# vitoplantamura/OnnxStream

Measured on AMD Instinct MI355X. Metric: sd15_unet_step_latency_ms+images_per_sec_512x512_20step, higher is better.
Workload: dtype f16

## Files before the change

onnxstream_amd/csrc/osg_tchain.hip:

```cpp
#include "osg_common.h"

#include <cstdlib>
#include <type_traits>

namespace osg_tb {

struct TailParams {
    const f16 *a1, *x0;
    const f16 *wo1, *bo1;
    const f16 *g2, *be2;
    float eps2;
    const f16 *wq2, *bq2;
    const f16 *kp, *vtp;
    float sc_log2e;
    int Tk;
    const f16 *wo2, *bo2;
    const f16 *g3, *be3;
    float eps3;
    const f16 *w1, *b1, *w2, *b2;
    const f16 *wpo, *bpo, *xin;
    f16 *out, *out2;
    long ldo, ldo2;
    int M, rows_per_img, heads;
    int pf_sleep0, pf_sleep;
    f16* dbg[8];
};

typedef __attribute__((address_space(3))) void* lds_ptr;

__device__ __forceinline__ void lds_barrier() {
    asm volatile("s_waitcnt lgkmcnt(0)" ::: "memory");
    __builtin_amdgcn_s_barrier();
}


template <int I, int N, typename Fn>
__device__ __forceinline__ void static_for_impl(Fn&& f) {
    if constexpr (I < N) {
        f(std::integral_constant<int, I>{});
        static_for_impl<I + 1, N>(f);
    }
}
template <int N, typename Fn>
__device__ __forceinline__ void static_for(Fn&& f) { static_for_impl<0, N>(f); }

template <int RT>
constexpr int kTileBytes = RT * 2048;

template <int RT>
__device__ __forceinline__ int img_off(int m, int n) { return (n >> 6) * kTileBytes<RT> + m * 128 + ((((n & 63) >> 3) ^ (m & 7)) << 4) + (n & 7) * 2; }

typedef unsigned u32x4 __attribute__((ext_vector_type(4)));
__device__ __forceinline__ f16x8 ldb(__amdgpu_buffer_rsrc_t rs, unsigned lo, int so) {
    return __builtin_bit_cast(f16x8, __builtin_amdgcn_raw_buffer_load_b128(rs, lo, so, 0));
}
template <int NT>
__device__ __forceinline__ void load_b(f16x8 (&b)[10], __amdgpu_buffer_rsrc_t rs, unsigned lo, int so, int kstep) {
#pragma unroll
    for (int ks = 0; ks < 2; ks++)
#pragma unroll
        for (int j = 0; j < NT; j++) b[ks * 5 + j] = ldb(rs, lo, so + j * 256 + ks * kstep);
}
__device__ __forceinline__ void load_b_geglu(f16x8 (&b)[10], __amdgpu_buffer_rsrc_t rs, unsigned lo, int so, int kstep, int gate_off) {
#pragma unroll
    for (int ks = 0; ks < 2; ks++) {
#pragma unroll
        for (int j = 0; j < 4; j++) b[ks * 5 + j] = ldb(rs, lo, so + (j & 1) * 256 + (j >> 1) * gate_off + ks * kstep);
        b[ks * 5 + 4] = b[ks * 5 + 3];
    }
}

template <int RT, int NT>
__device__ __forceinline__ void mma_ktile(const char* At, int a_rd, const f16x8 (&b)[10], f32x4 (&acc)[RT][NT]) {
#pragma unroll
    for (int ks = 0; ks < 2; ks++) {
        f16x8 a[RT];
#pragma unroll
        for (int i = 0; i < RT; i++) a[i] = *reinterpret_cast<const f16x8*>(At + ((a_rd + i * 2048) ^ (ks << 6)));
#pragma unroll
        for (int j = 0; j < NT; j++)
#pragma unroll
            for (int i = 0; i < RT; i++) acc[i][j] = __builtin_amdgcn_mfma_f32_16x16x32_f16(b[ks * 5 + j], a[i], acc[i][j], 0, 0, 0);
    }
}

template <int RT, int KT, int NT, int SS, int NS, typename Load, typename Next, typename Mark>
__device__ __forceinline__ void gemm_stage(const char* A, int a_rd, f16x8 (&bq)[NS][10], f32x4 (&acc)[RT][NT], Load&& load, Next&& next, Mark&& mark) {
    static_for<KT>([&](auto tc) __attribute__((always_inline)) {
        constexpr int t = decltype(tc)::value;
        mark(t);
        if constexpr (t + NS - 1 < KT) load(bq[(SS + t + NS - 1) % NS], t + NS - 1);
        else next(bq[(SS + t + NS - 1) % NS], t + NS - 1 - KT);
        __builtin_amdgcn_sched_barrier(0);
        mma_ktile<RT, NT>(A + t * kTileBytes<RT>, a_rd, bq[(SS + t) % NS], acc);
        __builtin_amdgcn_sched_barrier(0);
    });
}

template <int RT, int KT, int NT, int SS, int NS, typename Load, typename Next>
__device__ __forceinline__ void gemm_stage(const char* A, int a_rd, f16x8 (&bq)[NS][10], f32x4 (&acc)[RT][NT], Load&& load, Next&& next) {
    gemm_stage<RT, KT, NT, SS, NS>(A, a_rd, bq, acc, load, next, [](int) __attribute__((always_inline)) {});
}

template <int RT, int KT, int NT, typename After, typename Mark>
__device__ __forceinline__ void square_stage(const char* A, int a_rd, f16x8 (&bs)[KT][10], f32x4 (&acc)[RT][NT], After&& after, Mark&& mark) {
    static_for<KT>([&](auto tc) __attribute__((always_inline)) {
        constexpr int t = decltype(tc)::value;
        mark(t);
        __builtin_amdgcn_sched_barrier(0);
        mma_ktile<RT, NT>(A + t * kTileBytes<RT>, a_rd, bs[t], acc);
        __builtin_amdgcn_sched_barrier(0);
        after(bs[t], t);
    });
}

template <int RT, int NT>
__device__ __forceinline__ void zero_acc(f32x4 (&acc)[RT][NT]) {
#pragma unroll
    for (int i = 0; i < RT; i++)
#pragma unroll
        for (int j = 0; j < NT; j++) acc[i][j] = f32x4{0.f, 0.f, 0.f, 0.f};
}

template <int RT, int NT, bool RES>
__device__ __forceinline__ void epi_to_lds(const f32x4 (&acc)[RT][NT], const char* bias, int nb, const char* res, char* dst, int lane) {
    const int l16 = lane & 15, g4 = (lane >> 4) * 4;
#pragma unroll
    for (int j = 0; j < NT; j++) {
        const int n = nb + j * 16 + g4;
        const f16x4 bv = *reinterpret_cast<const f16x4*>(bias + n * 2);
#pragma unroll
        for (int i = 0; i < RT; i++) {
            const int off = img_off<RT>(i * 16 + l16, n);
            f16x4 rv = f16x4{0, 0, 0, 0};
            if constexpr (RES) rv = *reinterpret_cast<const f16x4*>(res + off);
            f16x4 o;
#pragma unroll
            for (int r = 0; r < 4; r++) o[r] = (f16)((acc[i][j][r] + (float)bv[r]) + (float)rv[r]);
            *reinterpret_cast<f16x4*>(dst + off) = o;
        }
    }
}

template <int RT, int NT, bool RES_LDS, bool OUT2>
__device__ __forceinline__ void epi_to_global(const f32x4 (&acc)[RT][NT], const char* bias, int nb, const char* res_lds, const f16x4 (&rg)[RT][NT],
                                              f16* __restrict__ out, long ldo, f16* __restrict__ out2, long ldo2, long row0, int lane) {
    const int l16 = lane & 15, g4 = (lane >> 4) * 4;
#pragma unroll
    for (int j = 0; j < NT; j++) {
        const int n = nb + j * 16 + g4;
        const f16x4 bv = *reinterpret_cast<const f16x4*>(bias + n * 2);
#pragma unroll
        for (int i = 0; i < RT; i++) {
            const int m = i * 16 + l16;
            f16x4 rv = rg[i][j];
            if constexpr (RES_LDS) rv = *reinterpret_cast<const f16x4*>(res_lds + img_off<RT>(m, n));
            f16x4 o;
#pragma unroll
            for (int r = 0; r < 4; r++) o[r] = (f16)((acc[i][j][r] + (float)bv[r]) + (float)rv[r]);
            *reinterpret_cast<f16x4*>(out + (row0 + m) * ldo + n) = o;
            if constexpr (OUT2) *reinterpret_cast<f16x4*>(out2 + (row0 + m) * ldo2 + n) = o;
        }
    }
}

template <int RT, int C>
__device__ __forceinline__ void ln_rows(const char* X, char* P, const char* gamma, const char* beta, float eps, int tid) {
    constexpr int NCH = C / 8, LPR = 16 / RT, PER = NCH / LPR;
    static_assert(NCH % LPR == 0 && (LPR == 4 || LPR == 8), "row chunks split over the lanes of a row");
    const int row = tid / LPR, part = tid % LPR;
    float v[PER][8];
    float s = 0.f;
#pragma unroll
    for (int i = 0; i < PER; i++) {
        const int c = part + LPR * i;
        const f16x8 t = *reinterpret_cast<const f16x8*>(X + (c >> 3) * kTileBytes<RT> + row * 128 + (((c & 7) ^ (row & 7)) << 4));
#pragma unroll
        for (int e = 0; e < 8; e++) { v[i][e] = (float)t[e]; s += v[i][e]; }
    }
    s += __shfl_xor(s, 1, 64);
    s += __shfl_xor(s, 2, 64);
    if constexpr (LPR == 8) s += __shfl_xor(s, 4, 64);
    const float mean = s / (float)C;
    float q = 0.f;
#pragma unroll
    for (int i = 0; i < PER; i++)
#pragma unroll
        for (int e = 0; e < 8; e++) { const float d = v[i][e] - mean; q += d * d; }
    q += __shfl_xor(q, 1, 64);
    q += __shfl_xor(q, 2, 64);
    if constexpr (LPR == 8) q += __shfl_xor(q, 4, 64);
    const float rstd = 1.0f / sqrtf(q / (float)C + eps);
#pragma unroll
    for (int i = 0; i < PER; i++) {
        const int c = part + LPR * i;
        const f16x8 gm = *reinterpret_cast<const f16x8*>(gamma + c * 16);
        const f16x8 bt = *reinterpret_cast<const f16x8*>(beta + c * 16);
        f16x8 o;
#pragma unroll
        for (int e = 0; e < 8; e++) o[e] = (f16)((v[i][e] - mean) * rstd * (float)gm[e] + (float)bt[e]);
        *reinterpret_cast<f16x8*>(P + (c >> 3) * kTileBytes<RT> + row * 128 + (((c & 7) ^ (row & 7)) << 4)) = o;
    }
}

template <int RT, int C>
__device__ __forceinline__ void dump_img(const char* img, f16* __restrict__ dst, long row0, int tid) {
    if (!dst) return;
    constexpr int NCH = C / 8;
    for (int idx = tid; idx < 16 * RT * NCH; idx += 256) {
        const int row = idx / NCH, c = idx - row * NCH;
        *reinterpret_cast<f16x8*>(dst + (row0 + row) * C + c * 8) =
            *reinterpret_cast<const f16x8*>(img + (c >> 3) * kTileBytes<RT> + row * 128 + (((c & 7) ^ (row & 7)) << 4));
    }
}

template <int RT, int D, int TKT>
__device__ __forceinline__ void cross_attention(const char* Qi, char* Oi, const f16* __restrict__ kp, const f16* __restrict__ vtp, int head0, int nheads, float c, int Tk, int lane) {
    constexpr int DS = (D + 15) / 16, DP = DS * 16, TKP = TKT * 16;
    const int l16 = lane & 15, g = lane >> 4;
    for (int hh = 0; hh < nheads; hh++) {
        const int h = head0 + hh;
        const f16* kh = kp + (long)h * TKP * DP;
        const f16* vh = vtp + (long)h * DP * TKP;
        f16x4 kf[TKT][DS], vf[DS][TKT];
#pragma unroll
        for (int tt = 0; tt < TKT; tt++)
#pragma unroll
            for (int ds = 0; ds < DS; ds++) kf[tt][ds] = *reinterpret_cast<const f16x4*>(kh + (tt * 16 + l16) * DP + ds * 16 + g * 4);
#pragma unroll
        for (int dt = 0; dt < DS; dt++)
#pragma unroll
            for (int tt = 0; tt < TKT; tt++) vf[dt][tt] = *reinterpret_cast<const f16x4*>(vh + (dt * 16 + l16) * TKP + tt * 16 + g * 4);
#pragma unroll 1
        for (int mi = 0; mi < RT; mi++) {
            const int m = mi * 16 + l16;
            f16x4 qf[DS];
#pragma unroll
            for (int ds = 0; ds < DS; ds++) {
                const int dd = ds * 16 + g * 4;
                const bool ok = dd < D;
                const f16x4 t = *reinterpret_cast<const f16x4*>(Qi + img_off<RT>(m, h * D + (ok ? dd : 0)));
                qf[ds] = ok ? t : f16x4{0, 0, 0, 0};
            }
            f32x4 s[TKT];
#pragma unroll
            for (int tt = 0; tt < TKT; tt++) {
                s[tt] = f32x4{0.f, 0.f, 0.f, 0.f};
#pragma unroll
                for (int ds = 0; ds < DS; ds++) s[tt] = __builtin_amdgcn_mfma_f32_16x16x16f16(kf[tt][ds], qf[ds], s[tt], 0, 0, 0);
            }
            float mx = -INFINITY;
#pragma unroll
            for (int tt = 0; tt < TKT; tt++)
#pragma unroll
                for (int r = 0; r < 4; r++) {
                    const float v = (tt * 16 + g * 4 + r) < Tk ? s[tt][r] * c : -INFINITY;
                    s[tt][r] = v;
                    mx = fmaxf(mx, v);
                }
            mx = fmaxf(mx, __shfl_xor(mx, 16, 64));
            mx = fmaxf(mx, __shfl_xor(mx, 32, 64));
            float sum = 0.f;
            f16x4 pf[TKT];
#pragma unroll
            for (int tt = 0; tt < TKT; tt++)
#pragma unroll
                for (int r = 0; r < 4; r++) {
                    const float e = __builtin_amdgcn_exp2f(s[tt][r] - mx);
                    sum += e;
                    pf[tt][r] = (f16)e;
                }
            sum += __shfl_xor(sum, 16, 64);
            sum += __shfl_xor(sum, 32, 64);
            const float inv = 1.0f / sum;
#pragma unroll
            for (int dt = 0; dt < DS; dt++) {
                f32x4 o = f32x4{0.f, 0.f, 0.f, 0.f};
#pragma unroll
                for (int tt = 0; tt < TKT; tt++) o = __builtin_amdgcn_mfma_f32_16x16x16f16(vf[dt][tt], pf[tt], o, 0, 0, 0);
                const int dd = dt * 16 + g * 4;
                if (dd < D) {
                    f16x4 ov;
#pragma unroll
                    for (int r = 0; r < 4; r++) ov[r] = (f16)(o[r] * inv);
                    *reinterpret_cast<f16x4*>(Oi + img_off<RT>(m, h * D + dd)) = ov;
                }
            }
        }
    }
}

__device__ __forceinline__ void touch_lines(const void* base, int rows, int row_bytes, long pitch, int tid, char* lds_dummy) {
    const int lpr = (row_bytes + 127) >> 7, n = rows * lpr;
    __amdgpu_buffer_rsrc_t rs = __builtin_amdgcn_make_buffer_rsrc((void*)base, 0, (int)((rows - 1) * pitch + row_bytes), 0x00020000);
    for (int i = tid; i < n; i += 256) {
        const int r = i / lpr, l = i - r * lpr;
        __builtin_amdgcn_raw_ptr_buffer_load_lds(rs, (lds_ptr)lds_dummy, 4, (unsigned)(r * pitch + l * 128), 0, 0, 0);
    }
}

template <int RT, int C, int D, int TKT, int NS>
__global__ __launch_bounds__(256, RT == 2 && NS == 2 ? 2 : 1) void tblock_tail_kernel(const void* a1, const void* x0, const void* wo1, const void* bo1, const void* g2, const void* be2, int M, int rows_per_img, TailParams pk) {
    TailParams p = pk;
    p.a1 = (const f16*)a1; p.x0 = (const f16*)x0; p.wo1 = (const f16*)wo1; p.bo1 = (const f16*)bo1; p.g2 = (const f16*)g2; p.be2 = (const f16*)be2; p.M = M; p.rows_per_img = rows_per_img;
    constexpr int RB = 16 * RT;
    constexpr int TB = kTileBytes<RT>;
    constexpr int KT = C / 64;
    constexpr int NTW = C / 64;
    constexpr int F = 4 * C;
    constexpr int HC = 128, NCHUNK = F / HC;
    constexpr int G2T = HC / 64;
    constexpr int PER = KT + G2T;
    constexpr int IMG = KT * TB;
    constexpr int AH = NS - 1;
    static_assert(C % 64 == 0 && NTW <= 5 && 2 * G2T * TB <= IMG && (RT == 2 || RT == 4) && (NS == 2 || NS == 3) && PER % NS == 1 && AH <= G2T && AH <= KT, "shape");
    constexpr int KS_C = 4 * C * 16, KT_C = 8 * C * 16, KS_1 = 4 * 2 * F * 16, KT_1 = 8 * 2 * F * 16;
    constexpr int GATE = F * 16;
    constexpr int CH1 = HC * 16;
    constexpr int CH2 = (HC / 8) * C * 16;
    const int tid = threadIdx.x;
    const int nblk = p.M / RB;

    if ((int)blockIdx.x >= nblk) {
        extern __shared__ __attribute__((aligned(16))) char lds_pf[];
        char* dummy = lds_pf + __builtin_amdgcn_readfirstlane(tid >> 6) * 256;
        auto nap = [&](int n) __attribute__((always_inline)) { for (; n > 0; n -= 127) __builtin_amdgcn_s_sleep(127); };
        touch_lines(p.wq2, 1, C * C * 2, 0, tid, dummy);
        {
            constexpr int DP = (D + 15) / 16 * 16;
            const int imgs = p.M / p.rows_per_img, bytes = imgs * p.heads * TKT * 16 * DP * 2;
            touch_lines(p.kp, 1, bytes, 0, tid, dummy);
            touch_lines(p.vtp, 1, bytes, 0, tid, dummy);
        }
        touch_lines(p.wo2, 1, C * C * 2, 0, tid, dummy);
        nap(p.pf_sleep0);
        for (int c = 0; c < NCHUNK; c++) {
            touch_lines((const char*)p.w1 + c * CH1, C / 8, HC * 16, 2 * F * 16, tid, dummy);
            touch_lines((const char*)p.w1 + GATE + c * CH1, C / 8, HC * 16, 2 * F * 16, tid, dummy);
            touch_lines((const char*)p.w2 + c * CH2, 1, CH2, 0, tid, dummy);
            if (c == NCHUNK / 2 && p.wpo) touch_lines(p.wpo, 1, C * C * 2, 0, tid, dummy);
            nap(p.pf_sleep);
        }
        return;
    }

    extern __shared__ __attribute__((aligned(16))) char lds[];
    char* const X = lds;
    char* const P = lds + IMG;
    char* const R = lds + 2 * IMG;
    char* const VEC = lds + 3 * IMG;
    enum { V_BO1, V_G2, V_BE2, V_BQ2, V_BO2, V_G3, V_BE3, V_B2, V_BPO, V_B1 };
    auto vec = [&](int k) __attribute__((always_inline)) { return VEC + k * (C * 2); };
    {
        const f16* src[10] = {p.bo1, p.g2, p.be2, p.bq2, p.bo2, p.g3, p.be3, p.b2, p.bpo, p.b1};
#pragma unroll
        for (int k = 0; k < 10; k++) {
            const int n16 = (k == V_B1 ? 2 * F : C) / 8;
            for (int i = tid; i < n16; i += 256) {
                f16x8 v = f16x8{0, 0, 0, 0, 0, 0, 0, 0};
                if (src[k]) v = *reinterpret_cast<const f16x8*>(src[k] + i * 8);
                *reinterpret_cast<f16x8*>(vec(k) + i * 16) = v;
            }
        }
    }
    const int lane = tid & 63;
    const int wave = __builtin_amdgcn_readfirstlane(tid >> 6);
    const int l16 = lane & 15, g = lane >> 4;
    const long row0 = (long)blockIdx.x * RB;
    const int img = (int)(row0 / p.rows_per_img);
    const int a_rd = l16 * 128 + ((g ^ (l16 & 7)) << 4);
    const int nb = wave * (C / 4);
    long long* const stamps = reinterpret_cast<long long*>(p.dbg[7]);
    auto stamp = [&](int k) __attribute__((always_inline)) { if (stamps && tid == 0) stamps[(long)blockIdx.x * 32 + k] = wall_clock64(); };
    stamp(0);

    f16x8 bq[NS][10];
    f16x8 bs[KT][10];
    const unsigned lo_c = (unsigned)((g * C + nb + l16) * 16);
    const unsigned lo_1 = (unsigned)((g * 2 * F + wave * 32 + l16) * 16);
    const __amdgpu_buffer_rsrc_t u_o1 = __builtin_amdgcn_make_buffer_rsrc((void*)p.wo1, 0, C * C * 2, 0x00020000);
    const __amdgpu_buffer_rsrc_t u_q2 = __builtin_amdgcn_make_buffer_rsrc((void*)p.wq2, 0, C * C * 2, 0x00020000);
    const __amdgpu_buffer_rsrc_t u_o2 = __builtin_amdgcn_make_buffer_rsrc((void*)p.wo2, 0, C * C * 2, 0x00020000);
    const __amdgpu_buffer_rsrc_t u_1 = __builtin_amdgcn_make_buffer_rsrc((void*)p.w1, 0, 2 * F * C * 2, 0x00020000);
    const __amdgpu_buffer_rsrc_t u_2 = __builtin_amdgcn_make_buffer_rsrc((void*)p.w2, 0, C * F * 2, 0x00020000);
    const __amdgpu_buffer_rsrc_t u_po = __builtin_amdgcn_make_buffer_rsrc((void*)p.wpo, 0, p.wpo ? C * C * 2 : 0, 0x00020000);
    const bool has_po = p.wpo != nullptr;
    auto ld_cc = [&](f16x8 (&b)[10], __amdgpu_buffer_rsrc_t rs, int t) __attribute__((always_inline)) { load_b<NTW>(b, rs, lo_c, t * KT_C, KS_C); };
    auto ld_ff = [&](f16x8 (&b)[10], int cc, int pos) __attribute__((always_inline)) {
        if (pos < KT) load_b_geglu(b, u_1, lo_1, cc * CH1 + pos * KT_1, KS_1, GATE);
        else load_b<NTW>(b, u_2, lo_c, (cc - 1) * CH2 + (pos - KT) * KT_C, KS_C);
    };

    static_for<KT>([&](auto tc) __attribute__((always_inline)) { ld_cc(bs[decltype(tc)::value], u_o1, decltype(tc)::value); });

    {
        __amdgpu_buffer_rsrc_t rsA = __builtin_amdgcn_make_buffer_rsrc((void*)(p.a1 + row0 * C), 0, RB * C * 2, 0x00020000);
        __amdgpu_buffer_rsrc_t rsX = __builtin_amdgcn_make_buffer_rsrc((void*)(p.x0 + row0 * C), 0, RB * C * 2, 0x00020000);
        const int rsub = lane >> 3, gch = (lane & 7) ^ rsub;
#pragma unroll
        for (int kt = 0; kt < KT; kt++)
#pragma unroll
            for (int qq = 0; qq < RT / 2; qq++) {
                const int q8 = qq * 4 + wave;
                const unsigned off = (unsigned)(((q8 * 8 + rsub) * C + kt * 64 + gch * 8) * 2);
                __builtin_amdgcn_raw_ptr_buffer_load_lds(rsA, (lds_ptr)(P + kt * TB + q8 * 1024), 16, off, 0, 0, 0);
                __builtin_amdgcn_raw_ptr_buffer_load_lds(rsX, (lds_ptr)(X + kt * TB + q8 * 1024), 16, off, 0, 0, 0);
            }
    }
    asm volatile("s_waitcnt vmcnt(0)" ::: "memory");
    lds_barrier();
    stamp(1);

    {
        f32x4 acc[RT][NTW];
        zero_acc(acc);
        square_stage<RT, KT, NTW>(P, a_rd, bs, acc, [&](f16x8 (&)[10], int t) __attribute__((always_inline)) { if (t < AH) ld_cc(bq[t % NS], u_q2, t); },
                              [&](int t) __attribute__((always_inline)) { stamp(16 + t); });
        stamp(21);
        epi_to_lds<RT, NTW, true>(acc, vec(V_BO1), nb, X, X, lane);
        stamp(22);
    }
    lds_barrier();
    stamp(2);
    dump_img<RT, C>(X, p.dbg[0], row0, tid);
    ln_rows<RT, C>(X, P, vec(V_G2), vec(V_BE2), p.eps2, tid);
    lds_barrier();
    stamp(3);
    dump_img<RT, C>(P, p.dbg[1], row0, tid);

    {
        f32x4 acc[RT][NTW];
        zero_acc(acc);
        gemm_stage<RT, KT, NTW, 0, NS>(P, a_rd, bq, acc, [&](f16x8 (&b)[10], int t) __attribute__((always_inline)) { ld_cc(b, u_q2, t); },
                                   [&](f16x8 (&b)[10], int j) __attribute__((always_inline)) { ld_cc(b, u_o2, j); });
        epi_to_lds<RT, NTW, false>(acc, vec(V_BQ2), nb, nullptr, R, lane);
    }
    lds_barrier();
    stamp(4);
    dump_img<RT, C>(R, p.dbg[2], row0, tid);

    {
        constexpr int DS = (D + 15) / 16, DP = DS * 16, TKP = TKT * 16;
        const int hpw = p.heads >> 2;
        const long per_img = (long)p.heads * TKP * DP;
        cross_attention<RT, D, TKT>(R, P, p.kp + img * per_img, p.vtp + img * per_img, wave * hpw, hpw, p.sc_log2e, p.Tk, lane);
    }
    lds_barrier();
    stamp(5);
    dump_img<RT, C>(P, p.dbg[3], row0, tid);

    {
        f32x4 acc[RT][NTW];
        zero_acc(acc);
        gemm_stage<RT, KT, NTW, KT, NS>(P, a_rd, bq, acc, [&](f16x8 (&b)[10], int t) __attribute__((always_inline)) { ld_cc(b, u_o2, t); },
                                    [&](f16x8 (&b)[10], int j) __attribute__((always_inline)) { ld_ff(b, 0, j); });
        epi_to_lds<RT, NTW, true>(acc, vec(V_BO2), nb, X, X, lane);
    }
    lds_barrier();
    stamp(6);
    dump_img<RT, C>(X, p.dbg[4], row0, tid);
    ln_rows<RT, C>(X, P, vec(V_G3), vec(V_BE3), p.eps3, tid);
    lds_barrier();
    stamp(7);
    dump_img<RT, C>(P, p.dbg[5], row0, tid);

    f32x4 accY[RT][NTW];
    zero_acc(accY);
    {
        constexpr int S0 = 2 * KT;
        f32x4 accG[RT][4];
        auto geglu_store = [&](int c) __attribute__((always_inline)) {
            char* H = R + (c & 1) * (G2T * TB);
#pragma unroll
            for (int jt = 0; jt < 2; jt++) {
                const int hc = wave * 32 + jt * 16 + g * 4;
                const f16x4 bv = *reinterpret_cast<const f16x4*>(vec(V_B1) + (c * HC + hc) * 2);
                const f16x4 bg = *reinterpret_cast<const f16x4*>(vec(V_B1) + (F + c * HC + hc) * 2);
#pragma unroll
                for (int i = 0; i < RT; i++) {
                    f16x4 o;
#pragma unroll
                    for (int r = 0; r < 4; r++) o[r] = (f16)((accG[i][jt][r] + (float)bv[r]) * osg_gelu_erf(accG[i][2 + jt][r] + (float)bg[r]));
                    *reinterpret_cast<f16x4*>(H + img_off<RT>(i * 16 + l16, hc)) = o;
                }
            }
        };
        zero_acc(accG);
        gemm_stage<RT, KT, 4, S0, NS>(P, a_rd, bq, accG, [&](f16x8 (&b)[10], int t) __attribute__((always_inline)) { ld_ff(b, 0, t); },
                                  [&](f16x8 (&b)[10], int j) __attribute__((always_inline)) { ld_ff(b, 1, j); });
        geglu_store(0);
        lds_barrier();
        stamp(8);
        auto ff_iter = [&](auto st, int c) __attribute__((always_inline)) {
            constexpr int ST = decltype(st)::value;
            const bool last = c == NCHUNK - 1;
            auto request = [&](f16x8 (&b)[10], int pos) __attribute__((always_inline)) {
                if (pos < PER) ld_ff(b, c, pos);
                else if (!last) ld_ff(b, c + 1, pos - PER);
                else ld_ff(b, NCHUNK, KT + pos - PER);
            };
            zero_acc(accG);
            static_for<KT>([&](auto tc) __attribute__((always_inline)) {
                constexpr int t = decltype(tc)::value;
                request(bq[(ST + t + AH) % NS], t + AH);
                __builtin_amdgcn_sched_barrier(0);
                mma_ktile<RT, 4>(P + t * TB, a_rd, bq[(ST + t) % NS], accG);
                __builtin_amdgcn_sched_barrier(0);
            });
            if (c == 3) stamp(24); else if (c == 4) stamp(28);
            const char* Hp = R + ((c - 1) & 1) * (G2T * TB);
            static_for<G2T>([&](auto uc) __attribute__((always_inline)) {
                constexpr int u = decltype(uc)::value;
                request(bq[(ST + KT + u + AH) % NS], KT + u + AH);
                __builtin_amdgcn_sched_barrier(0);
                mma_ktile<RT, NTW>(Hp + u * TB, a_rd, bq[(ST + KT + u) % NS], accY);
            });
            if (c == 3) stamp(25); else if (c == 4) stamp(29);
            geglu_store(c);
            if (c == 3) stamp(26); else if (c == 4) stamp(30);
            lds_barrier();
            if (c == 2) stamp(23); else if (c == 3) stamp(27); else if (c == 4) stamp(31);
        };
        constexpr int B0 = (S0 + KT) % NS;
        int c = 1;
        for (; c + NS <= NCHUNK; c += NS) {
            ff_iter(std::integral_constant<int, B0 % NS>{}, c);
            ff_iter(std::integral_constant<int, (B0 + 1) % NS>{}, c + 1);
            if constexpr (NS == 3) ff_iter(std::integral_constant<int, (B0 + 2) % NS>{}, c + 2);
        }
        constexpr int REM = (NCHUNK - 1) % NS;
        if constexpr (REM >= 1) ff_iter(std::integral_constant<int, B0 % NS>{}, c);
        if constexpr (REM >= 2) ff_iter(std::integral_constant<int, (B0 + 1) % NS>{}, c + 1);
        stamp(9);
        {
            constexpr int ST = (S0 + KT + (NCHUNK - 1) * PER) % NS;
            const char* Hp = R + ((NCHUNK - 1) & 1) * (G2T * TB);
            static_for<G2T>([&](auto uc) __attribute__((always_inline)) {
                constexpr int u = decltype(uc)::value;
                if constexpr (u + AH < G2T) ld_ff(bq[(ST + u + AH) % NS], NCHUNK, KT + u + AH);
                else if (has_po) ld_cc(bq[(ST + u + AH) % NS], u_po, u + AH - G2T);
                __builtin_amdgcn_sched_barrier(0);
                mma_ktile<RT, NTW>(Hp + u * TB, a_rd, bq[(ST + u) % NS], accY);
                __builtin_amdgcn_sched_barrier(0);
            });
        }
    }
    stamp(10);
    f16x4 rg[RT][NTW];
#pragma unroll
    for (int i = 0; i < RT; i++)
#pragma unroll
        for (int j = 0; j < NTW; j++) rg[i][j] = f16x4{0, 0, 0, 0};
    if (!has_po) {
        if (p.out2) epi_to_global<RT, NTW, true, true>(accY, vec(V_B2), nb, X, rg, p.out, p.ldo, p.out2, p.ldo2, row0, lane);
        else epi_to_global<RT, NTW, true, false>(accY, vec(V_B2), nb, X, rg, p.out, p.ldo, nullptr, 0, row0, lane);
        if (stamps) { asm volatile("s_waitcnt vmcnt(0)" ::: "memory"); stamp(13); }
        return;
    }
#pragma unroll
    for (int i = 0; i < RT; i++)
#pragma unroll
        for (int j = 0; j < NTW; j++) rg[i][j] = *reinterpret_cast<const f16x4*>(p.xin + (row0 + i * 16 + l16) * C + nb + j * 16 + g * 4);
    epi_to_lds<RT, NTW, true>(accY, vec(V_B2), nb, X, P, lane);
    lds_barrier();
    stamp(11);
    dump_img<RT, C>(P, p.dbg[6], row0, tid);
    {
        f32x4 acc[RT][NTW];
        zero_acc(acc);
        constexpr int SS = 2 * KT + KT + (NCHUNK - 1) * PER + G2T;
        gemm_stage<RT, KT, NTW, SS, NS>(P, a_rd, bq, acc, [&](f16x8 (&b)[10], int t) __attribute__((always_inline)) { ld_cc(b, u_po, t); },
                                    [&](f16x8 (&)[10], int) __attribute__((always_inline)) {});
        stamp(12);
        if (p.out2) epi_to_global<RT, NTW, false, true>(acc, vec(V_BPO), nb, nullptr, rg, p.out, p.ldo, p.out2, p.ldo2, row0, lane);
        else epi_to_global<RT, NTW, false, false>(acc, vec(V_BPO), nb, nullptr, rg, p.out, p.ldo, nullptr, 0, row0, lane);
        if (stamps) { asm volatile("s_waitcnt vmcnt(0)" ::: "memory"); stamp(13); }
    }
}

struct PackJob { int k_col, v_col, D, dst; };
__global__ __launch_bounds__(256) void kv_pack_kernel(const f16* __restrict__ base, long ld, int Tk, int heads, int imgs, const PackJob* __restrict__ jobs, f16* __restrict__ dst) {
    const int per_job = imgs * heads;
    const int j = blockIdx.x / per_job, ih = blockIdx.x - j * per_job, img = ih / heads, h = ih - img * heads;
    const PackJob job = jobs[j];
    const int D = job.D, DP = (D + 15) / 16 * 16, TKP = 80, NC = DP / 8;
    f16* kp = dst + job.dst + (long)ih * TKP * DP;
    f16* vtp = dst + job.dst + (long)per_job * TKP * DP + (long)ih * TKP * DP;
    const f16* k = base + job.k_col + h * D + (long)img * Tk * ld;
    const f16* v = base + job.v_col + h * D + (long)img * Tk * ld;
    for (int idx = threadIdx.x; idx < TKP * NC; idx += 256) {
        const int t = idx / NC, d0 = (idx - t * NC) * 8;
        const bool in = t < Tk && d0 < D;
        f16x8 kv = f16x8{0, 0, 0, 0, 0, 0, 0, 0}, vv = kv;
        if (in) {
            kv = *reinterpret_cast<const f16x8*>(k + (long)t * ld + d0);
            vv = *reinterpret_cast<const f16x8*>(v + (long)t * ld + d0);
        }
        *reinterpret_cast<f16x8*>(kp + t * DP + d0) = kv;
#pragma unroll
        for (int e = 0; e < 8; e++) vtp[(d0 + e) * TKP + t] = vv[e];
    }
}

__global__ __launch_bounds__(256) void kn8_pack_kernel(const f16x8* __restrict__ src, f16x8* __restrict__ dst, int N, int K8) {
    const long idx = (long)blockIdx.x * 256 + threadIdx.x;
    if (idx >= (long)N * K8) return;
    const int kc = (int)(idx / N), n = (int)(idx - (long)kc * N);
    dst[idx] = src[(long)n * K8 + kc];
}


}

extern "C" {

int osg_tblock_tail_supported(int M, int rows_per_img, int C, int heads, int Tk) {
    return C == 320 && heads == 8 && M > 0 && M % 32 == 0 && rows_per_img % 32 == 0 && Tk >= 1 && Tk <= 80;
}

size_t osg_tblock_kv_pack_elems(int imgs, int heads, int D) { return (size_t)imgs * heads * 80 * (size_t)((D + 15) / 16 * 16); }

int osg_tblock_pack_weight(osg_ctx* ctx, const void* w_nk, int N, int K, void* w_kn8) {
    if (N < 1 || K < 8 || K % 8) OSG_FAIL(ctx, "osg_tblock_pack_weight: K must be a multiple of 8");
    const long n = (long)N * (K / 8);
    hipLaunchKernelGGL(osg_tb::kn8_pack_kernel, dim3((unsigned)((n + 255) / 256)), dim3(256), 0, ctx->compute, (const f16x8*)w_nk, (f16x8*)w_kn8, N, K / 8);
    OSG_LAUNCH_CHECK(ctx);
    return 0;
}

int osg_tblock_kv_pack_jobs(osg_ctx* ctx, const void* base, long ld, int imgs, int Tk, int heads, int njobs, const int* jobs_dev, void* dst) {
    if (Tk < 1 || Tk > 80 || njobs < 1 || imgs < 1 || heads < 1 || ld % 8) OSG_FAIL(ctx, "osg_tblock_kv_pack_jobs: unsupported shape (1 <= Tk <= 80, row pitch a multiple of 8 elements; columns and head dims multiples of 8)");
    hipLaunchKernelGGL(osg_tb::kv_pack_kernel, dim3((unsigned)(njobs * imgs * heads)), dim3(256), 0, ctx->compute, (const f16*)base, ld, Tk, heads, imgs,
                       (const osg_tb::PackJob*)jobs_dev, (f16*)dst);
    OSG_LAUNCH_CHECK(ctx);
    return 0;
}

int osg_tblock_tail(osg_ctx* ctx, const osg_tblock_tail_args* a) {
    if (!osg_tblock_tail_supported(a->M, a->rows_per_img, a->C, a->heads, a->Tk)) OSG_FAIL(ctx, "osg_tblock_tail: unsupported shape (see osg_tblock_tail_supported)");
    if (!(a->scale > 0.f)) OSG_FAIL(ctx, "osg_tblock_tail: scale must be > 0");
    if (!a->a1 || !a->x0 || !a->wo1 || !a->g2 || !a->be2 || !a->wq2 || !a->kp || !a->vtp || !a->wo2 || !a->g3 || !a->be3 || !a->w1 || !a->w2 || !a->out)
        OSG_FAIL(ctx, "osg_tblock_tail: missing operand");
    if (a->wpo && !a->xin) OSG_FAIL(ctx, "osg_tblock_tail: proj_out needs its residual");
    osg_tb::TailParams p;
    p.a1 = (const f16*)a->a1; p.x0 = (const f16*)a->x0;
    p.wo1 = (const f16*)a->wo1; p.bo1 = (const f16*)a->bo1;
    p.g2 = (const f16*)a->g2; p.be2 = (const f16*)a->be2; p.eps2 = a->eps2;
    p.wq2 = (const f16*)a->wq2; p.bq2 = (const f16*)a->bq2;
    p.kp = (const f16*)a->kp; p.vtp = (const f16*)a->vtp;
    p.sc_log2e = a->scale * 1.4426950408889634f;
    p.Tk = a->Tk;
    p.wo2 = (const f16*)a->wo2; p.bo2 = (const f16*)a->bo2;
    p.g3 = (const f16*)a->g3; p.be3 = (const f16*)a->be3; p.eps3 = a->eps3;
    p.w1 = (const f16*)a->w1; p.b1 = (const f16*)a->b1; p.w2 = (const f16*)a->w2; p.b2 = (const f16*)a->b2;
    p.wpo = (const f16*)a->wpo; p.bpo = (const f16*)a->bpo; p.xin = (const f16*)a->xin;
    p.out = (f16*)a->out; p.out2 = (f16*)a->out2;
    p.ldo = a->ldo ? a->ldo : a->C; p.ldo2 = a->ldo2;
    p.M = a->M; p.rows_per_img = a->rows_per_img; p.heads = a->heads;
    for (int i = 0; i < 8; i++) p.dbg[i] = (f16*)a->dbg[i];
    static const int pfw = getenv("OSG_TBLOCK_PREFETCH") ? atoi(getenv("OSG_TBLOCK_PREFETCH")) : 8;
    static const int pfs0 = getenv("OSG_TBLOCK_PF_SLEEP0") ? atoi(getenv("OSG_TBLOCK_PF_SLEEP0")) : 100;
    static const int pfs = getenv("OSG_TBLOCK_PF_SLEEP") ? atoi(getenv("OSG_TBLOCK_PF_SLEEP")) : 60;
    p.pf_sleep0 = pfs0; p.pf_sleep = pfs;
    static const int rows_env = getenv("OSG_TBLOCK_ROWS") ? atoi(getenv("OSG_TBLOCK_ROWS")) : 0;
    int rows = a->rows_per_block == 32 || a->rows_per_block == 64 ? a->rows_per_block : rows_env == 32 || rows_env == 64 ? rows_env : (a->M / 64 < 2 * ctx->num_cu ? 32 : 64);
    if (a->rows_per_block != 0 && a->rows_per_block != 32 && a->rows_per_block != 64) OSG_FAIL(ctx, "osg_tblock_tail: rows_per_block must be 0, 32 or 64");
    if (a->M % 64 || a->rows_per_img % 64) {
        if (a->rows_per_block == 64) OSG_FAIL(ctx, "osg_tblock_tail: 64-row blocks need M and rows_per_img to be multiples of 64");
        rows = 32;
    }
    const int nblk = a->M / rows;
    const int npf = nblk >= 64 && nblk + pfw <= ctx->num_cu ? pfw : 0;
    auto launch = [&](auto kern, int smem, unsigned long long& attr_mask) -> int {
        if (osg_first_on_device(attr_mask)) {
            OSG_HIP(ctx, hipFuncSetAttribute((const void*)kern, hipFuncAttributeMaxDynamicSharedMemorySize, smem));
        }
        hipLaunchKernelGGL(kern, dim3((unsigned)(nblk + npf)), dim3(256), smem, ctx->compute, (const void*)p.a1, (const void*)p.x0, (const void*)p.wo1, (const void*)p.bo1, (const void*)p.g2, (const void*)p.be2, p.M, p.rows_per_img, p);
        return 0;
    };
    constexpr int vec_bytes = (9 * 320 + 8 * 320) * 2;
    static unsigned long long attr64 = 0, attr32 = 0, attr32n3 = 0;
    static const bool ns3 = getenv("OSG_TBLOCK_NS") && atoi(getenv("OSG_TBLOCK_NS")) == 3;
    int rc;
    if (rows == 64) rc = launch(osg_tb::tblock_tail_kernel<4, 320, 40, 5, 2>, 3 * 5 * osg_tb::kTileBytes<4> + vec_bytes, attr64);
    else if (ns3) rc = launch(osg_tb::tblock_tail_kernel<2, 320, 40, 5, 3>, 3 * 5 * osg_tb::kTileBytes<2> + vec_bytes, attr32n3);
    else rc = launch(osg_tb::tblock_tail_kernel<2, 320, 40, 5, 2>, 3 * 5 * osg_tb::kTileBytes<2> + vec_bytes, attr32);
    if (rc) return rc;
    OSG_LAUNCH_CHECK(ctx);
    osg_set_kernel(ctx, 4, rows, rows == 32 && ns3 ? 3 : 2, nblk, npf, a->wpo ? 1 : 0, a->out2 ? 1 : 0);
    return 0;
}

}
```

Baseline: 10.34.

## Split FFN chunks across two wave groups in 32-row transformer tail kernel

Adds an NG=2 variant of the fused transformer-block tail kernel with 512 threads, used by default for 32-row blocks. The second group of four waves takes odd GEGLU/FFN chunks and half the cross-attention heads, and its FFN partial accumulators are reduced through LDS into group 0. The aim is more waves per block to hide weight-streaming latency in the FFN. In exchange, the non-FFN GEMMs leave group 1 idle, there are extra barriers and a reduction step, and per-block register/LDS demand rises, which may lower occupancy.

```diff
diff --git a/onnxstream_amd/csrc/osg_tchain.hip b/onnxstream_amd/csrc/osg_tchain.hip
--- a/onnxstream_amd/csrc/osg_tchain.hip
+++ b/onnxstream_amd/csrc/osg_tchain.hip
@@ -203,11 +203,11 @@
     }
 }
 
-template <int RT, int C>
+template <int RT, int C, int NTH>
 __device__ __forceinline__ void dump_img(const char* img, f16* __restrict__ dst, long row0, int tid) {
     if (!dst) return;
     constexpr int NCH = C / 8;
-    for (int idx = tid; idx < 16 * RT * NCH; idx += 256) {
+    for (int idx = tid; idx < 16 * RT * NCH; idx += NTH) {
         const int row = idx / NCH, c = idx - row * NCH;
         *reinterpret_cast<f16x8*>(dst + (row0 + row) * C + c * 8) =
             *reinterpret_cast<const f16x8*>(img + (c >> 3) * kTileBytes<RT> + row * 128 + (((c & 7) ^ (row & 7)) << 4));
@@ -290,17 +290,18 @@
     }
 }
 
+template <int NTH>
 __device__ __forceinline__ void touch_lines(const void* base, int rows, int row_bytes, long pitch, int tid, char* lds_dummy) {
     const int lpr = (row_bytes + 127) >> 7, n = rows * lpr;
     __amdgpu_buffer_rsrc_t rs = __builtin_amdgcn_make_buffer_rsrc((void*)base, 0, (int)((rows - 1) * pitch + row_bytes), 0x00020000);
-    for (int i = tid; i < n; i += 256) {
+    for (int i = tid; i < n; i += NTH) {
         const int r = i / lpr, l = i - r * lpr;
         __builtin_amdgcn_raw_ptr_buffer_load_lds(rs, (lds_ptr)lds_dummy, 4, (unsigned)(r * pitch + l * 128), 0, 0, 0);
     }
 }
 
-template <int RT, int C, int D, int TKT, int NS>
-__global__ __launch_bounds__(256, RT == 2 && NS == 2 ? 2 : 1) void tblock_tail_kernel(const void* a1, const void* x0, const void* wo1, const void* bo1, const void* g2, const void* be2, int M, int rows_per_img, TailParams pk) {
+template <int RT, int C, int D, int TKT, int NS, int NG = 1>
+__global__ __launch_bounds__(256 * NG, RT == 2 && NS == 2 ? 2 : 1) void tblock_tail_kernel(const void* a1, const void* x0, const void* wo1, const void* bo1, const void* g2, const void* be2, int M, int rows_per_img, TailParams pk) {
     TailParams p = pk;
     p.a1 = (const f16*)a1; p.x0 = (const f16*)x0; p.wo1 = (const f16*)wo1; p.bo1 = (const f16*)bo1; p.g2 = (const f16*)g2; p.be2 = (const f16*)be2; p.M = M; p.rows_per_img = rows_per_img;
     constexpr int RB = 16 * RT;
@@ -313,7 +314,13 @@
     constexpr int PER = KT + G2T;
     constexpr int IMG = KT * TB;
     constexpr int AH = NS - 1;
+    constexpr int NTH = 256 * NG;
+    constexpr int CS = NG;
+    constexpr int NITER = NCHUNK / CS;
+    constexpr int SUMB = RT * NTW * 256 * 16;
+    constexpr int RSZ = NG == 2 ? SUMB : IMG;
     static_assert(C % 64 == 0 && NTW <= 5 && 2 * G2T * TB <= IMG && (RT == 2 || RT == 4) && (NS == 2 || NS == 3) && PER % NS == 1 && AH <= G2T && AH <= KT, "shape");
+    static_assert((NG == 1 || NG == 2) && NCHUNK % CS == 0 && RSZ >= IMG && RSZ >= NG * 2 * G2T * TB && (NG == 1 || RT == 2), "wave groups");
     constexpr int KS_C = 4 * C * 16, KT_C = 8 * C * 16, KS_1 = 4 * 2 * F * 16, KT_1 = 8 * 2 * F * 16;
     constexpr int GATE = F * 16;
     constexpr int CH1 = HC * 16;
@@ -325,20 +332,20 @@
         extern __shared__ __attribute__((aligned(16))) char lds_pf[];
         char* dummy = lds_pf + __builtin_amdgcn_readfirstlane(tid >> 6) * 256;
         auto nap = [&](int n) __attribute__((always_inline)) { for (; n > 0; n -= 127) __builtin_amdgcn_s_sleep(127); };
-        touch_lines(p.wq2, 1, C * C * 2, 0, tid, dummy);
+        touch_lines<NTH>(p.wq2, 1, C * C * 2, 0, tid, dummy);
         {
             constexpr int DP = (D + 15) / 16 * 16;
             const int imgs = p.M / p.rows_per_img, bytes = imgs * p.heads * TKT * 16 * DP * 2;
-            touch_lines(p.kp, 1, bytes, 0, tid, dummy);
-            touch_lines(p.vtp, 1, bytes, 0, tid, dummy);
-        }
-        touch_lines(p.wo2, 1, C * C * 2, 0, tid, dummy);
+            touch_lines<NTH>(p.kp, 1, bytes, 0, tid, dummy);
+            touch_lines<NTH>(p.vtp, 1, bytes, 0, tid, dummy);
+        }
+        touch_lines<NTH>(p.wo2, 1, C * C * 2, 0, tid, dummy);
         nap(p.pf_sleep0);
         for (int c = 0; c < NCHUNK; c++) {
-            touch_lines((const char*)p.w1 + c * CH1, C / 8, HC * 16, 2 * F * 16, tid, dummy);
-            touch_lines((const char*)p.w1 + GATE + c * CH1, C / 8, HC * 16, 2 * F * 16, tid, dummy);
-            touch_lines((const char*)p.w2 + c * CH2, 1, CH2, 0, tid, dummy);
-            if (c == NCHUNK / 2 && p.wpo) touch_lines(p.wpo, 1, C * C * 2, 0, tid, dummy);
+            touch_lines<NTH>((const char*)p.w1 + c * CH1, C / 8, HC * 16, 2 * F * 16, tid, dummy);
+            touch_lines<NTH>((const char*)p.w1 + GATE + c * CH1, C / 8, HC * 16, 2 * F * 16, tid, dummy);
+            touch_lines<NTH>((const char*)p.w2 + c * CH2, 1, CH2, 0, tid, dummy);
+            if (c == NCHUNK / 2 && p.wpo) touch_lines<NTH>(p.wpo, 1, C * C * 2, 0, tid, dummy);
             nap(p.pf_sleep);
         }
         return;
@@ -348,7 +355,7 @@
     char* const X = lds;
     char* const P = lds + IMG;
     char* const R = lds + 2 * IMG;
-    char* const VEC = lds + 3 * IMG;
+    char* const VEC = lds + 2 * IMG + RSZ;
     enum { V_BO1, V_G2, V_BE2, V_BQ2, V_BO2, V_G3, V_BE3, V_B2, V_BPO, V_B1 };
     auto vec = [&](int k) __attribute__((always_inline)) { return VEC + k * (C * 2); };
     {
@@ -356,7 +363,7 @@
 #pragma unroll
         for (int k = 0; k < 10; k++) {
             const int n16 = (k == V_B1 ? 2 * F : C) / 8;
-            for (int i = tid; i < n16; i += 256) {
+            for (int i = tid; i < n16; i += NTH) {
                 f16x8 v = f16x8{0, 0, 0, 0, 0, 0, 0, 0};
                 if (src[k]) v = *reinterpret_cast<const f16x8*>(src[k] + i * 8);
                 *reinterpret_cast<f16x8*>(vec(k) + i * 16) = v;
@@ -365,11 +372,14 @@
     }
     const int lane = tid & 63;
     const int wave = __builtin_amdgcn_readfirstlane(tid >> 6);
+    const int grp = NG == 2 ? wave >> 2 : 0;
+    const int w4 = NG == 2 ? wave & 3 : wave;
+    const bool g0 = grp == 0;
     const int l16 = lane & 15, g = lane >> 4;
     const long row0 = (long)blockIdx.x * RB;
     const int img = (int)(row0 / p.rows_per_img);
     const int a_rd = l16 * 128 + ((g ^ (l16 & 7)) << 4);
-    const int nb = wave * (C / 4);
+    const int nb = w4 * (C / 4);
     long long* const stamps = reinterpret_cast<long long*>(p.dbg[7]);
     auto stamp = [&](int k) __attribute__((always_inline)) { if (stamps && tid == 0) stamps[(long)blockIdx.x * 32 + k] = wall_clock64(); };
     stamp(0);
@@ -377,7 +387,7 @@
     f16x8 bq[NS][10];
     f16x8 bs[KT][10];
     const unsigned lo_c = (unsigned)((g * C + nb + l16) * 16);
-    const unsigned lo_1 = (unsigned)((g * 2 * F + wave * 32 + l16) * 16);
+    const unsigned lo_1 = (unsigned)((g * 2 * F + w4 * 32 + l16) * 16);
     const __amdgpu_buffer_rsrc_t u_o1 = __builtin_amdgcn_make_buffer_rsrc((void*)p.wo1, 0, C * C * 2, 0x00020000);
     const __amdgpu_buffer_rsrc_t u_q2 = __builtin_amdgcn_make_buffer_rsrc((void*)p.wq2, 0, C * C * 2, 0x00020000);
     const __amdgpu_buffer_rsrc_t u_o2 = __builtin_amdgcn_make_buffer_rsrc((void*)p.wo2, 0, C * C * 2, 0x00020000);
@@ -388,10 +398,10 @@
     auto ld_cc = [&](f16x8 (&b)[10], __amdgpu_buffer_rsrc_t rs, int t) __attribute__((always_inline)) { load_b<NTW>(b, rs, lo_c, t * KT_C, KS_C); };
     auto ld_ff = [&](f16x8 (&b)[10], int cc, int pos) __attribute__((always_inline)) {
         if (pos < KT) load_b_geglu(b, u_1, lo_1, cc * CH1 + pos * KT_1, KS_1, GATE);
-        else load_b<NTW>(b, u_2, lo_c, (cc - 1) * CH2 + (pos - KT) * KT_C, KS_C);
+        else load_b<NTW>(b, u_2, lo_c, (cc - CS) * CH2 + (pos - KT) * KT_C, KS_C);
     };
 
-    static_for<KT>([&](auto tc) __attribute__((always_inline)) { ld_cc(bs[decltype(tc)::value], u_o1, decltype(tc)::value); });
+    if (g0) static_for<KT>([&](auto tc) __attribute__((always_inline)) { ld_cc(bs[decltype(tc)::value], u_o1, decltype(tc)::value); });
 
     {
         __amdgpu_buffer_rsrc_t rsA = __builtin_amdgcn_make_buffer_rsrc((void*)(p.a1 + row0 * C), 0, RB * C * 2, 0x00020000);
@@ -401,20 +411,23 @@
         for (int kt = 0; kt < KT; kt++)
 #pragma unroll
             for (int qq = 0; qq < RT / 2; qq++) {
-                const int q8 = qq * 4 + wave;
+                const int q8 = qq * 4 + w4;
                 const unsigned off = (unsigned)(((q8 * 8 + rsub) * C + kt * 64 + gch * 8) * 2);
-                __builtin_amdgcn_raw_ptr_buffer_load_lds(rsA, (lds_ptr)(P + kt * TB + q8 * 1024), 16, off, 0, 0, 0);
-                __builtin_amdgcn_raw_ptr_buffer_load_lds(rsX, (lds_ptr)(X + kt * TB + q8 * 1024), 16, off, 0, 0, 0);
+                if (NG == 1 || g0) __builtin_amdgcn_raw_ptr_buffer_load_lds(rsA, (lds_ptr)(P + kt * TB + q8 * 1024), 16, off, 0, 0, 0);
+                if (NG == 1 || !g0) __builtin_amdgcn_raw_ptr_buffer_load_lds(rsX, (lds_ptr)(X + kt * TB + q8 * 1024), 16, off, 0, 0, 0);
             }
     }
     asm volatile("s_waitcnt vmcnt(0)" ::: "memory");
     lds_barrier();
     stamp(1);
 
-    {
+    if (g0) {
         f32x4 acc[RT][NTW];
         zero_acc(acc);
-        square_stage<RT, KT, NTW>(P, a_rd, bs, acc, [&](f16x8 (&)[10], int t) __attribute__((always_inline)) { if (t < AH) ld_cc(bq[t % NS], u_q2, t); },
+        square_stage<RT, KT, NTW>(P, a_rd, bs, acc, [&](f16x8 (&)[10], int t) __attribute__((always_inline)) {
+                                  constexpr int DL = NG == 2 ? 1 : 0;
+                                  if (t >= DL && t - DL < AH) ld_cc(bq[(t - DL) % NS], u_q2, t - DL);
+                              },
                               [&](int t) __attribute__((always_inline)) { stamp(16 + t); });
         stamp(21);
         epi_to_lds<RT, NTW, true>(acc, vec(V_BO1), nb, X, X, lane);
@@ -422,13 +435,13 @@
     }
     lds_barrier();
     stamp(2);
-    dump_img<RT, C>(X, p.dbg[0], row0, tid);
-    ln_rows<RT, C>(X, P, vec(V_G2), vec(V_BE2), p.eps2, tid);
+    dump_img<RT, C, NTH>(X, p.dbg[0], row0, tid);
+    if (g0) ln_rows<RT, C>(X, P, vec(V_G2), vec(V_BE2), p.eps2, tid);
     lds_barrier();
     stamp(3);
-    dump_img<RT, C>(P, p.dbg[1], row0, tid);
-
-    {
+    dump_img<RT, C, NTH>(P, p.dbg[1], row0, tid);
+
+    if (g0) {
         f32x4 acc[RT][NTW];
         zero_acc(acc);
         gemm_stage<RT, KT, NTW, 0, NS>(P, a_rd, bq, acc, [&](f16x8 (&b)[10], int t) __attribute__((always_inline)) { ld_cc(b, u_q2, t); },
@@ -437,43 +450,46 @@
     }
     lds_barrier();
     stamp(4);
-    dump_img<RT, C>(R, p.dbg[2], row0, tid);
+    dump_img<RT, C, NTH>(R, p.dbg[2], row0, tid);
 
     {
         constexpr int DS = (D + 15) / 16, DP = DS * 16, TKP = TKT * 16;
-        const int hpw = p.heads >> 2;
+        const int hpw = p.heads >> (NG == 2 ? 3 : 2);
         const long per_img = (long)p.heads * TKP * DP;
         cross_attention<RT, D, TKT>(R, P, p.kp + img * per_img, p.vtp + img * per_img, wave * hpw, hpw, p.sc_log2e, p.Tk, lane);
     }
     lds_barrier();
     stamp(5);
-    dump_img<RT, C>(P, p.dbg[3], row0, tid);
-
-    {
+    dump_img<RT, C, NTH>(P, p.dbg[3], row0, tid);
+
+    if (g0) {
         f32x4 acc[RT][NTW];
         zero_acc(acc);
         gemm_stage<RT, KT, NTW, KT, NS>(P, a_rd, bq, acc, [&](f16x8 (&b)[10], int t) __attribute__((always_inline)) { ld_cc(b, u_o2, t); },
                                     [&](f16x8 (&b)[10], int j) __attribute__((always_inline)) { ld_ff(b, 0, j); });
         epi_to_lds<RT, NTW, true>(acc, vec(V_BO2), nb, X, X, lane);
+    } else {
+        static_for<AH>([&](auto jc) __attribute__((always_inline)) { ld_ff(bq[(2 * KT + decltype(jc)::value) % NS], grp, decltype(jc)::value); });
     }
     lds_barrier();
     stamp(6);
-    dump_img<RT, C>(X, p.dbg[4], row0, tid);
-    ln_rows<RT, C>(X, P, vec(V_G3), vec(V_BE3), p.eps3, tid);
+    dump_img<RT, C, NTH>(X, p.dbg[4], row0, tid);
+    if (g0) ln_rows<RT, C>(X, P, vec(V_G3), vec(V_BE3), p.eps3, tid);
     lds_barrier();
     stamp(7);
-    dump_img<RT, C>(P, p.dbg[5], row0, tid);
+    dump_img<RT, C, NTH>(P, p.dbg[5], row0, tid);
 
     f32x4 accY[RT][NTW];
     zero_acc(accY);
     {
         constexpr int S0 = 2 * KT;
         f32x4 accG[RT][4];
+        auto hbuf = [&](int c) __attribute__((always_inline)) { return R + (NG == 2 ? grp * 2 + ((c >> 1) & 1) : c & 1) * (G2T * TB); };
         auto geglu_store = [&](int c) __attribute__((always_inline)) {
-            char* H = R + (c & 1) * (G2T * TB);
+            char* H = hbuf(c);
 #pragma unroll
             for (int jt = 0; jt < 2; jt++) {
-                const int hc = wave * 32 + jt * 16 + g * 4;
+                const int hc = w4 * 32 + jt * 16 + g * 4;
                 const f16x4 bv = *reinterpret_cast<const f16x4*>(vec(V_B1) + (c * HC + hc) * 2);
                 const f16x4 bg = *reinterpret_cast<const f16x4*>(vec(V_B1) + (F + c * HC + hc) * 2);
 #pragma unroll
@@ -486,18 +502,19 @@
             }
         };
         zero_acc(accG);
-        gemm_stage<RT, KT, 4, S0, NS>(P, a_rd, bq, accG, [&](f16x8 (&b)[10], int t) __attribute__((always_inline)) { ld_ff(b, 0, t); },
-                                  [&](f16x8 (&b)[10], int j) __attribute__((always_inline)) { ld_ff(b, 1, j); });
-        geglu_store(0);
+        gemm_stage<RT, KT, 4, S0, NS>(P, a_rd, bq, accG, [&](f16x8 (&b)[10], int t) __attribute__((always_inline)) { ld_ff(b, grp, t); },
+                                  [&](f16x8 (&b)[10], int j) __attribute__((always_inline)) { ld_ff(b, grp + CS, j); });
+        geglu_store(grp);
         lds_barrier();
         stamp(8);
-        auto ff_iter = [&](auto st, int c) __attribute__((always_inline)) {
+        auto ff_iter = [&](auto st, int k) __attribute__((always_inline)) {
             constexpr int ST = decltype(st)::value;
-            const bool last = c == NCHUNK - 1;
+            const int c = grp + k * CS;
+            const bool last = k == NITER - 1;
             auto request = [&](f16x8 (&b)[10], int pos) __attribute__((always_inline)) {
                 if (pos < PER) ld_ff(b, c, pos);
-                else if (!last) ld_ff(b, c + 1, pos - PER);
-                else ld_ff(b, NCHUNK, KT + pos - PER);
+                else if (!last) ld_ff(b, c + CS, pos - PER);
+                else ld_ff(b, NG == 1 ? NCHUNK : c + CS, KT + pos - PER);
             };
             zero_acc(accG);
             static_for<KT>([&](auto tc) __attribute__((always_inline)) {
@@ -507,38 +524,39 @@
                 mma_ktile<RT, 4>(P + t * TB, a_rd, bq[(ST + t) % NS], accG);
                 __builtin_amdgcn_sched_barrier(0);
             });
-            if (c == 3) stamp(24); else if (c == 4) stamp(28);
-            const char* Hp = R + ((c - 1) & 1) * (G2T * TB);
+            if ((NG == 1 ? c : k) == 3) stamp(24); else if ((NG == 1 ? c : k) == 4) stamp(28);
+            const char* Hp = hbuf(c - CS);
             static_for<G2T>([&](auto uc) __attribute__((always_inline)) {
                 constexpr int u = decltype(uc)::value;
                 request(bq[(ST + KT + u + AH) % NS], KT + u + AH);
                 __builtin_amdgcn_sched_barrier(0);
                 mma_ktile<RT, NTW>(Hp + u * TB, a_rd, bq[(ST + KT + u) % NS], accY);
             });
-            if (c == 3) stamp(25); else if (c == 4) stamp(29);
+            if ((NG == 1 ? c : k) == 3) stamp(25); else if ((NG == 1 ? c : k) == 4) stamp(29);
             geglu_store(c);
-            if (c == 3) stamp(26); else if (c == 4) stamp(30);
+            if ((NG == 1 ? c : k) == 3) stamp(26); else if ((NG == 1 ? c : k) == 4) stamp(30);
             lds_barrier();
-            if (c == 2) stamp(23); else if (c == 3) stamp(27); else if (c == 4) stamp(31);
+            if ((NG == 1 ? c : k) == 2) stamp(23); else if ((NG == 1 ? c : k) == 3) stamp(27); else if ((NG == 1 ? c : k) == 4) stamp(31);
         };
         constexpr int B0 = (S0 + KT) % NS;
-        int c = 1;
-        for (; c + NS <= NCHUNK; c += NS) {
-            ff_iter(std::integral_constant<int, B0 % NS>{}, c);
-            ff_iter(std::integral_constant<int, (B0 + 1) % NS>{}, c + 1);
-            if constexpr (NS == 3) ff_iter(std::integral_constant<int, (B0 + 2) % NS>{}, c + 2);
-        }
-        constexpr int REM = (NCHUNK - 1) % NS;
-        if constexpr (REM >= 1) ff_iter(std::integral_constant<int, B0 % NS>{}, c);
-        if constexpr (REM >= 2) ff_iter(std::integral_constant<int, (B0 + 1) % NS>{}, c + 1);
+        int k = 1;
+        for (; k + NS <= NITER; k += NS) {
+            ff_iter(std::integral_constant<int, B0 % NS>{}, k);
+            ff_iter(std::integral_constant<int, (B0 + 1) % NS>{}, k + 1);
+            if constexpr (NS == 3) ff_iter(std::integral_constant<int, (B0 + 2) % NS>{}, k + 2);
+        }
+        constexpr int REM = (NITER - 1) % NS;
+        if constexpr (REM >= 1) ff_iter(std::integral_constant<int, B0 % NS>{}, k);
+        if constexpr (REM >= 2) ff_iter(std::integral_constant<int, (B0 + 1) % NS>{}, k + 1);
         stamp(9);
         {
-            constexpr int ST = (S0 + KT + (NCHUNK - 1) * PER) % NS;
-            const char* Hp = R + ((NCHUNK - 1) & 1) * (G2T * TB);
+            constexpr int ST = (S0 + KT + (NITER - 1) * PER) % NS;
+            const int cl = grp + (NITER - 1) * CS;
+            const char* Hp = hbuf(cl);
             static_for<G2T>([&](auto uc) __attribute__((always_inline)) {
                 constexpr int u = decltype(uc)::value;
-                if constexpr (u + AH < G2T) ld_ff(bq[(ST + u + AH) % NS], NCHUNK, KT + u + AH);
-                else if (has_po) ld_cc(bq[(ST + u + AH) % NS], u_po, u + AH - G2T);
+                if constexpr (u + AH < G2T) ld_ff(bq[(ST + u + AH) % NS], cl + CS, KT + u + AH);
+                else if (has_po && g0) ld_cc(bq[(ST + u + AH) % NS], u_po, u + AH - G2T);
                 __builtin_amdgcn_sched_barrier(0);
                 mma_ktile<RT, NTW>(Hp + u * TB, a_rd, bq[(ST + u) % NS], accY);
                 __builtin_amdgcn_sched_barrier(0);
@@ -546,29 +564,49 @@
         }
     }
     stamp(10);
+    if constexpr (NG == 2) {
+        lds_barrier();
+        if (!g0) {
+#pragma unroll
+            for (int i = 0; i < RT; i++)
+#pragma unroll
+                for (int j = 0; j < NTW; j++) *reinterpret_cast<f32x4*>(R + ((i * NTW + j) * 256 + w4 * 64 + lane) * 16) = accY[i][j];
+        }
+        lds_barrier();
+        if (g0) {
+#pragma unroll
+            for (int i = 0; i < RT; i++)
+#pragma unroll
+                for (int j = 0; j < NTW; j++) accY[i][j] = accY[i][j] + *reinterpret_cast<const f32x4*>(R + ((i * NTW + j) * 256 + w4 * 64 + lane) * 16);
+        }
+        stamp(14);
+    }
     f16x4 rg[RT][NTW];
 #pragma unroll
     for (int i = 0; i < RT; i++)
 #pragma unroll
         for (int j = 0; j < NTW; j++) rg[i][j] = f16x4{0, 0, 0, 0};
     if (!has_po) {
+        if (!g0) return;
         if (p.out2) epi_to_global<RT, NTW, true, true>(accY, vec(V_B2), nb, X, rg, p.out, p.ldo, p.out2, p.ldo2, row0, lane);
         else epi_to_global<RT, NTW, true, false>(accY, vec(V_B2), nb, X, rg, p.out, p.ldo, nullptr, 0, row0, lane);
         if (stamps) { asm volatile("s_waitcnt vmcnt(0)" ::: "memory"); stamp(13); }
         return;
     }
-#pragma unroll
-    for (int i = 0; i < RT; i++)
-#pragma unroll
-        for (int j = 0; j < NTW; j++) rg[i][j] = *reinterpret_cast<const f16x4*>(p.xin + (row0 + i * 16 + l16) * C + nb + j * 16 + g * 4);
-    epi_to_lds<RT, NTW, true>(accY, vec(V_B2), nb, X, P, lane);
+    if (g0) {
+#pragma unroll
+        for (int i = 0; i < RT; i++)
+#pragma unroll
+            for (int j = 0; j < NTW; j++) rg[i][j] = *reinterpret_cast<const f16x4*>(p.xin + (row0 + i * 16 + l16) * C + nb + j * 16 + g * 4);
+        epi_to_lds<RT, NTW, true>(accY, vec(V_B2), nb, X, P, lane);
+    }
     lds_barrier();
     stamp(11);
-    dump_img<RT, C>(P, p.dbg[6], row0, tid);
-    {
+    dump_img<RT, C, NTH>(P, p.dbg[6], row0, tid);
+    if (g0) {
         f32x4 acc[RT][NTW];
         zero_acc(acc);
-        constexpr int SS = 2 * KT + KT + (NCHUNK - 1) * PER + G2T;
+        constexpr int SS = 2 * KT + KT + (NITER - 1) * PER + G2T;
         gemm_stage<RT, KT, NTW, SS, NS>(P, a_rd, bq, acc, [&](f16x8 (&b)[10], int t) __attribute__((always_inline)) { ld_cc(b, u_po, t); },
                                     [&](f16x8 (&)[10], int) __attribute__((always_inline)) {});
         stamp(12);
@@ -671,20 +709,23 @@
     }
     const int nblk = a->M / rows;
     const int npf = nblk >= 64 && nblk + pfw <= ctx->num_cu ? pfw : 0;
-    auto launch = [&](auto kern, int smem, unsigned long long& attr_mask) -> int {
+    auto launch = [&](auto kern, int threads, int smem, unsigned long long& attr_mask) -> int {
         if (osg_first_on_device(attr_mask)) {
             OSG_HIP(ctx, hipFuncSetAttribute((const void*)kern, hipFuncAttributeMaxDynamicSharedMemorySize, smem));
         }
-        hipLaunchKernelGGL(kern, dim3((unsigned)(nblk + npf)), dim3(256), smem, ctx->compute, (const void*)p.a1, (const void*)p.x0, (const void*)p.wo1, (const void*)p.bo1, (const void*)p.g2, (const void*)p.be2, p.M, p.rows_per_img, p);
+        hipLaunchKernelGGL(kern, dim3((unsigned)(nblk + npf)), dim3((unsigned)threads), smem, ctx->compute, (const void*)p.a1, (const void*)p.x0, (const void*)p.wo1, (const void*)p.bo1, (const void*)p.g2, (const void*)p.be2, p.M, p.rows_per_img, p);
         return 0;
     };
     constexpr int vec_bytes = (9 * 320 + 8 * 320) * 2;
-    static unsigned long long attr64 = 0, attr32 = 0, attr32n3 = 0;
+    static unsigned long long attr64 = 0, attr32 = 0, attr32n3 = 0, attr32g2 = 0;
     static const bool ns3 = getenv("OSG_TBLOCK_NS") && atoi(getenv("OSG_TBLOCK_NS")) == 3;
+    const char* groups_env = getenv("OSG_TBLOCK_GROUPS");
+    const int groups = rows == 32 && !ns3 && !(groups_env && atoi(groups_env) == 1) ? 2 : 1;
     int rc;
-    if (rows == 64) rc = launch(osg_tb::tblock_tail_kernel<4, 320, 40, 5, 2>, 3 * 5 * osg_tb::kTileBytes<4> + vec_bytes, attr64);
-    else if (ns3) rc = launch(osg_tb::tblock_tail_kernel<2, 320, 40, 5, 3>, 3 * 5 * osg_tb::kTileBytes<2> + vec_bytes, attr32n3);
-    else rc = launch(osg_tb::tblock_tail_kernel<2, 320, 40, 5, 2>, 3 * 5 * osg_tb::kTileBytes<2> + vec_bytes, attr32);
+    if (rows == 64) rc = launch(osg_tb::tblock_tail_kernel<4, 320, 40, 5, 2>, 256, 3 * 5 * osg_tb::kTileBytes<4> + vec_bytes, attr64);
+    else if (ns3) rc = launch(osg_tb::tblock_tail_kernel<2, 320, 40, 5, 3>, 256, 3 * 5 * osg_tb::kTileBytes<2> + vec_bytes, attr32n3);
+    else if (groups == 2) rc = launch(osg_tb::tblock_tail_kernel<2, 320, 40, 5, 2, 2>, 512, 2 * 5 * osg_tb::kTileBytes<2> + 2 * 5 * 256 * 16 + vec_bytes, attr32g2);
+    else rc = launch(osg_tb::tblock_tail_kernel<2, 320, 40, 5, 2>, 256, 3 * 5 * osg_tb::kTileBytes<2> + vec_bytes, attr32);
     if (rc) return rc;
     OSG_LAUNCH_CHECK(ctx);
     osg_set_kernel(ctx, 4, rows, rows == 32 && ns3 ? 3 : 2, nblk, npf, a->wpo ? 1 : 0, a->out2 ? 1 : 0);
```

New measurement: 10.43, median of 6. Within noise of the previous version (+0.9%).
